# REXJJ/depth-map-fusion-utils

Hardware: AMD Instinct MI355X
Metric: ray-voxel updates/sec (3D-DDA log-odds fusion, 512^3 grid, 640x480 depth) (higher is better)
Workload: dtype int32

## Files before the change

### depth-map-fusion-utils_amd/csrc/dmf_dda.hpp

```cpp
#pragma once
#include "dmf_internal.hpp"

namespace dmf {

constexpr int64_t kQ = 256;

__device__ inline int64_t clampi(int64_t v, int64_t lo, int64_t hi) { return v < lo ? lo : (v > hi ? hi : v); }
__device__ inline int32_t clamp32(int32_t v, int32_t lo, int32_t hi) { return v < lo ? lo : (v > hi ? hi : v); }

__device__ inline int32_t floor_sat32(double x) {
  const double f = floor(x);
  return fabs(f) < 9223372036854775808.0 ? (int32_t)fmin(fmax(f, -1073741824.0), 1073741824.0) : -(1 << 30);
}

__device__ inline void atomic_add_dev(int32_t* p, int32_t v) {
  __hip_atomic_fetch_add(p, v, __ATOMIC_RELAXED, __HIP_MEMORY_SCOPE_AGENT);
}

struct Tiles {
  uint32_t ny, nz;
};
__host__ __device__ inline Tiles tiles_of(const int n[3]) {
  return Tiles{(uint32_t)(n[1] + 1) >> 1, (uint32_t)(n[2] + 3) >> 2};
}
__host__ __device__ inline uint32_t tile_base(const Tiles& t, int tx, int ty, int tz) {
  return (((uint32_t)tx * t.ny + (uint32_t)ty) * t.nz + (uint32_t)tz) << 4;
}
__host__ __device__ inline uint32_t tiled_index(const Tiles& t, int x, int y, int z) {
  return tile_base(t, x >> 1, y >> 1, z >> 2) | (uint32_t)(((x & 1) << 3) | ((y & 1) << 2) | (z & 3));
}
inline size_t tiled_cells(const int n[3]) {
  return (size_t)((n[0] + 1) >> 1) * (size_t)((n[1] + 1) >> 1) * (size_t)((n[2] + 3) >> 2) * 16;
}

struct Ray {
  int c[3];
  int st[3];
  int32_t E01, E02, E12;
  int32_t K[3];
  int left;
  bool end_inside;
};
constexpr int32_t kNever = 1 << 30;

__device__ inline void dda_select(int32_t& E01, int32_t& E02, int32_t& E12, int32_t K0, int32_t K1, int32_t K2,
                                  bool& s0, bool& s1, bool& s2) {
  const bool b10 = E01 > 0;
  s2 = (b10 ? E12 : E02) > 0;
  s1 = !s2 && b10;
  s0 = !s2 && !b10;
  E01 += s0 ? K1 : (s1 ? -K0 : 0);
  E02 += s0 ? K2 : (s2 ? -K0 : 0);
  E12 += s1 ? K2 : (s2 ? -K1 : 0);
}

__device__ inline double grid_coord(const Geom& g, int a, float x) {
  const double t = (double)x - g.mn[a];
  return g.pow2 ? t * g.inv[a] : t / g.dl[a];
}

__device__ inline void grid_origin(const Geom& g, const float O[3], double go[3]) {
#pragma unroll
  for (int a = 0; a < 3; ++a) go[a] = grid_coord(g, a, O[a]);
}

__device__ inline bool dda_quantize_go(const Geom& g, const double go[3], const float E[3], bool end_inside,
                                       int64_t qs[3], int64_t qe[3]) {
  double ge[3], D[3];
#pragma unroll
  for (int a = 0; a < 3; ++a) {
    ge[a] = grid_coord(g, a, E[a]);
    D[a] = ge[a] - go[a];
  }
  double t0 = 0.0, t1 = 1.0;
#pragma unroll
  for (int a = 0; a < 3; ++a) {
    if (D[a] == 0.0) {
      if (go[a] < 0.0 || go[a] >= (double)g.n[a]) return false;
    } else if (end_inside) {
      if (D[a] > 0.0 ? go[a] < 0.0 : go[a] > (double)g.n[a]) {
        const double lo = (D[a] > 0.0 ? 0.0 - go[a] : (double)g.n[a] - go[a]) / D[a];
        if (lo > t0) t0 = lo;
      }
    } else {
      double ta = (0.0 - go[a]) / D[a];
      double tb = ((double)g.n[a] - go[a]) / D[a];
      if (ta > tb) { const double tt = ta; ta = tb; tb = tt; }
      if (ta > t0) t0 = ta;
      if (tb < t1) t1 = tb;
    }
  }
  if (end_inside) { t1 = 1.0; if (t0 > 1.0) t0 = 1.0; }
  if (t0 > t1) return false;
#pragma unroll
  for (int a = 0; a < 3; ++a) {
    const double gs = go[a] + t0 * D[a];
    const double gx = end_inside ? ge[a] : go[a] + t1 * D[a];
    const int32_t n = (int32_t)g.n[a], Q = (int32_t)kQ;
    const int32_t cs = clamp32(floor_sat32(gs), 0, n - 1);
    const int32_t ce = end_inside ? floor_sat32(ge[a]) : clamp32(floor_sat32(gx), 0, n - 1);
    qs[a] = clamp32(floor_sat32(gs * (double)kQ), cs * Q, cs * Q + Q - 1);
    qe[a] = clamp32(floor_sat32(gx * (double)kQ), ce * Q, ce * Q + Q - 1);
  }
  return true;
}

__device__ inline bool dda_quantize(const Geom& g, const float O[3], const float E[3], bool end_inside, int64_t qs[3],
                                    int64_t qe[3]) {
  double go[3];
  grid_origin(g, O, go);
  return dda_quantize_go(g, go, E, end_inside, qs, qe);
}

__device__ inline bool dda_setup(const Geom& g, const float O[3], const float E[3], bool end_inside, Ray& R) {
  int64_t qs[3], qe[3];
  if (!dda_quantize(g, O, E, end_inside, qs, qe)) return false;
  int64_t cs[3], ce[3];
#pragma unroll
  for (int a = 0; a < 3; ++a) {
    cs[a] = qs[a] / kQ;
    ce[a] = qe[a] / kQ;
  }
  int64_t adq[3], h[3];
#pragma unroll
  for (int a = 0; a < 3; ++a) {
    const int64_t dq = qe[a] - qs[a];
    adq[a] = dq < 0 ? -dq : dq;
    R.st[a] = ce[a] > cs[a] ? 1 : (ce[a] < cs[a] ? -1 : 0);
    h[a] = R.st[a] > 0 ? 2 * ((cs[a] + 1) * kQ - qs[a]) : 2 * (qs[a] - cs[a] * kQ) + 1;
    R.K[a] = (int32_t)(2 * kQ * adq[a]);
  }
  auto pair = [&](int a, int b) -> int32_t {
    if (R.st[a] && R.st[b]) return (int32_t)(h[a] * adq[b] - h[b] * adq[a]);
    return R.st[a] ? -kNever : (R.st[b] ? kNever : 0);
  };
  R.E01 = pair(0, 1);
  R.E02 = pair(0, 2);
  R.E12 = pair(1, 2);
  const int nsteps = (int)((ce[0] > cs[0] ? ce[0] - cs[0] : cs[0] - ce[0]) + (ce[1] > cs[1] ? ce[1] - cs[1] : cs[1] - ce[1]) +
                           (ce[2] > cs[2] ? ce[2] - cs[2] : cs[2] - ce[2]));
  R.c[0] = (int)cs[0];
  R.c[1] = (int)cs[1];
  R.c[2] = (int)cs[2];
  R.left = nsteps + 1;
  R.end_inside = end_inside;
  return true;
}

__device__ inline bool endpoint_inside(const Geom& g, const float E[3]) {
  const bool in = (E[0] >= g.vlo[0]) & (E[0] <= g.vhi[0]) & (E[1] >= g.vlo[1]) & (E[1] <= g.vhi[1]) &
                  (E[2] >= g.vlo[2]) & (E[2] <= g.vhi[2]);
  if (!in) return false;
  return valid_coords(g, bin_axis(g, 0, E[0]), bin_axis(g, 1, E[1]), bin_axis(g, 2, E[2]));
}

__device__ inline int pixel_ray(const Geom& g, const CamP& cam, const uint16_t* __restrict__ depth,
                                const PoseX* __restrict__ poses, int p, int r, int c, int dmin, int dmax, Ray& R,
                                bool& valid) {
  R.left = 0;
  valid = false;
  if (r >= cam.H || c >= cam.W) return 0;
  const int d = depth[((int64_t)p * cam.H + r) * cam.W + c];
  if (!(d >= dmin && d < dmax)) return 0;
  valid = true;
  const PoseX& T = poses[p];
  float pc[3], E[3];
  project(cam, r, c, d, pc);
  xform(T.f, pc[0], pc[1], pc[2], E);
  const bool inside = endpoint_inside(g, E);
  const float O[3] = {T.f[3], T.f[7], T.f[11]};
  if (!dda_setup(g, O, E, inside, R)) { R.left = 0; return 0; }
  return R.left;
}

__device__ inline bool pixel_quant_go(const Geom& g, const CamP& cam, int d, const float Tf[12], const double go[3],
                                      int r, int c, int dmin, int dmax, int64_t qs[3], int64_t qe[3], bool& inside,
                                      bool& valid) {
  valid = false;
  inside = false;
  if (d < 0 || !(d >= dmin && d < dmax)) return false;
  valid = true;
  float pc[3], E[3];
  project(cam, r, c, d, pc);
  xform(Tf, pc[0], pc[1], pc[2], E);
  inside = endpoint_inside(g, E);
  return dda_quantize_go(g, go, E, inside, qs, qe);
}

__device__ inline int pixel_depth(const CamP& cam, const uint16_t* __restrict__ depth, int p, int r, int c) {
  return (r >= cam.H || c >= cam.W) ? -1 : (int)depth[((int64_t)p * cam.H + r) * cam.W + c];
}

}
```

### depth-map-fusion-utils_amd/csrc/dmf_fuse.hip

```cpp
#include <algorithm>
#include <atomic>
#include <cmath>
#include <cstdlib>
#include <string>
#include <type_traits>

#include "dmf_brick.hpp"
#include "dmf_dda.hpp"
#include "dmf_host.hpp"

namespace dmf {

struct DepthSrc {
  CamP cam;
  const uint16_t* depth;
  const PoseX* poses;
  int dmin, dmax, packets_x;
  struct Frame { float Tf[12]; };
  struct Sample { int d, r, c; };
  __device__ void begin(const Geom& g, int p, Frame& f, double go[3]) const {
#pragma unroll
    for (int i = 0; i < 12; ++i) f.Tf[i] = poses[p].f[i];
    const float O[3] = {f.Tf[3], f.Tf[7], f.Tf[11]};
    grid_origin(g, O, go);
// ... 21 lines not shown
  int64_t N;
  struct Frame { bool live; };
  struct Sample { float E[3]; bool ok; };
  __device__ static bool finite3(const float v[3]) {
    return __builtin_isfinite(v[0]) & __builtin_isfinite(v[1]) & __builtin_isfinite(v[2]);
  }
  __device__ void origin(int p, float O[3]) const {
    const float* const o = origins + 3 * (int64_t)p;
    O[0] = o[0];
    O[1] = o[1];
    O[2] = o[2];
  }
  __device__ void begin(const Geom& g, int p, Frame& f, double go[3]) const {
    float O[3];
    origin(p, O);
    f.live = finite3(O);
    grid_origin(g, O, go);
  }
  __device__ Sample load(int p, int q, int l) const {
    Sample s;
    const int64_t i = (int64_t)q * 64 + l;
    s.ok = i < N;
    const float* const e = xyz + ((int64_t)p * N + (s.ok ? i : 0)) * 3;
    s.E[0] = e[0];
    s.E[1] = e[1];
    s.E[2] = e[2];
    return s;
  }
  __device__ bool quant(const Geom& g, const Frame& f, const double go[3], const Sample& s, int64_t qs[3],
                        int64_t qe[3], bool& inside, bool& valid) const {
    inside = false;
    valid = f.live & s.ok & finite3(s.E);
    if (!valid) return false;
    inside = endpoint_inside(g, s.E);
    return dda_quantize_go(g, go, s.E, inside, qs, qe);
  }
  __device__ int ray(const Geom& g, int p, int q, int l, Ray& R, bool& valid) const {
    float O[3];
    origin(p, O);
    const Sample s = load(p, q, l);
    R.left = 0;
    valid = finite3(O) && s.ok && finite3(s.E);
    if (!valid) return 0;
    if (!dda_setup(g, O, s.E, endpoint_inside(g, s.E), R)) { R.left = 0; return 0; }
    return R.left;
  }
};

__device__ inline void wave_stats(unsigned long long* stats, unsigned long long upd, unsigned long long ray,
                                  unsigned long long hit) {
  for (int o = 32; o > 0; o >>= 1) {
    upd += __shfl_down(upd, o, 64);
    ray += __shfl_down(ray, o, 64);
    hit += __shfl_down(hit, o, 64);
  }
  if ((threadIdx.x & 63) == 0) {
    if (upd) atomicAdd(&stats[0], upd);
    if (ray) atomicAdd(&stats[1], ray);
    if (hit) atomicAdd(&stats[2], hit);
  }
}


typedef unsigned short us2 __attribute__((ext_vector_type(2)));
__device__ inline uint32_t pkmax(uint32_t a, uint32_t b) {
  us2 x = __builtin_bit_cast(us2, a), y = __builtin_bit_cast(us2, b);
  return __builtin_bit_cast(uint32_t, __builtin_elementwise_max(x, y));
}
__device__ inline uint32_t wave_pkmax(uint32_t v) {
  v = pkmax(v, (uint32_t)__builtin_amdgcn_update_dpp(0, (int)v, 0x111, 0xf, 0xf, false));
  v = pkmax(v, (uint32_t)__builtin_amdgcn_update_dpp(0, (int)v, 0x112, 0xf, 0xf, false));
  v = pkmax(v, (uint32_t)__builtin_amdgcn_update_dpp(0, (int)v, 0x114, 0xf, 0xf, false));
  v = pkmax(v, (uint32_t)__builtin_amdgcn_update_dpp(0, (int)v, 0x118, 0xf, 0xf, false));
  v = pkmax(v, (uint32_t)__builtin_amdgcn_update_dpp(0, (int)v, 0x142, 0xa, 0xf, false));
  v = pkmax(v, (uint32_t)__builtin_amdgcn_update_dpp(0, (int)v, 0x143, 0xc, 0xf, false));
  return (uint32_t)__builtin_amdgcn_readlane((int)v, 63);
}

__device__ inline int lane_prefix(uint64_t mask) {
  return (int)__builtin_amdgcn_mbcnt_hi((uint32_t)(mask >> 32), __builtin_amdgcn_mbcnt_lo((uint32_t)mask, 0u));
}

__device__ inline int small_div(int i, int b, float rb, int& rem) {
  int q = (int)((float)i * rb);
  int r = i - q * b;
  if (r < 0) { --q; r += b; }
  if (r >= b) { ++q; r -= b; }
  rem = r;
  return q;
}

__device__ inline int popc(uint32_t v) { return __builtin_popcount(v); }
__device__ inline int popc(uint64_t v) { return __builtin_popcountll(v); }

template <int kS, int kBox, class Src>
__global__ __launch_bounds__(64) void k_fuse_l(Geom g, Src src, int32_t* __restrict__ hits,
                                               int32_t* __restrict__ misses,
                                               unsigned long long* __restrict__ stats) {
  static_assert(kS <= 31, "2-bit codes of up to 31 advances with a 64-bit field mask");
  using CodeT = typename std::conditional<(kS <= 15), uint32_t, uint64_t>::type;
  constexpr CodeT kOne = 1, kOdd = (CodeT)0x5555555555555555ull, kEven = (CodeT)0xAAAAAAAAAAAAAAAAull;
  static_assert(kBox % 256 == 0 && kBox <= 65536, "box scanned 256 cells per iteration, 16-bit indices");
  static_assert(kBox >= 64 * kS, "the non-zero list lives in the box");
  stats = stat_slot(stats);
  __shared__ __attribute__((aligned(16))) int box[kBox];
  uint32_t* nzl = (uint32_t*)box;
  const int l = threadIdx.x;
  for (int i = l; i < kBox; i += 64) box[i] = 0;
  const Tiles tl = tiles_of(g.n);
  Ray R;
  bool valid;
  const unsigned long long upd = (unsigned long long)src.ray(g, (int)blockIdx.y, (int)blockIdx.x, l, R, valid);
  const unsigned long long nvalid = valid ? 1 : 0, nhit = (R.left > 0 && R.end_inside) ? 1 : 0;
  int32_t E01 = R.E01, E02 = R.E02, E12 = R.E12;
  const int32_t K0 = R.K[0], K1 = R.K[1], K2 = R.K[2];
  const int st0 = R.st[0], st1 = R.st[1], st2 = R.st[2];
  int c0 = R.c[0], c1 = R.c[1], c2 = R.c[2], left = R.left;
  const bool end_inside = R.end_inside;
  const int rot = ((l & 7) + 3 * (l >> 3)) % kS;
  unsigned long long nflush = 0, nround_lds = 0, nround_direct = 0;
  while (__builtin_amdgcn_ballot_w64(left > 0)) {
    const int rem = left < kS ? left : kS;
// ... 171 lines not shown

constexpr uint32_t kHashEmpty = 0xffff0000u;
__device__ inline bool hash_add(uint32_t* tab, uint32_t mask, int shift, uint32_t b, uint32_t n) {
  uint32_t h = (b * 2654435761u) >> shift;
  for (uint32_t k = 0; k <= mask; ++k) {
    const uint32_t old = atomicCAS(&tab[h], kHashEmpty, b << 16 | n);
    if (old == kHashEmpty) return true;
    if ((old >> 16) == b) {
      atomicAdd(&tab[h], n);
      return true;
    }
    h = (h + 1) & mask;
  }
  return false;
}

__device__ inline void hash_add_first(uint32_t* tab, uint32_t mask, int shift, int b, uint32_t* ovf) {
  const int b0 = __builtin_amdgcn_readfirstlane(b);
  const uint64_t same = __builtin_amdgcn_ballot_w64(b == b0);
  const int l = (int)(threadIdx.x & 63);
  if (b == b0 && l != __builtin_ctzll(same)) return;
  const uint32_t n = b == b0 ? (uint32_t)__builtin_popcountll(same) : 1u;
  if (!hash_add(tab, mask, shift, (uint32_t)b, n)) *ovf = 1u;
}

template <class Src>
struct BkRaysArgs {
  Geom g;
  Src src;
  int packets_pose, wg_pose, span;
  BkGeom bg;
  ulonglong2* rays;
  uint64_t* paths;
  uint32_t* pose_cnt;
  uint32_t* wg_base;
  uint32_t* wg_list;
  int wgl_stride;
  unsigned long long* pose_pairs;
  unsigned long long* stats;
  uint32_t* ovl;
  int hash_log;
};

template <bool H16, bool HASH, class Src>
__device__ inline void bk_rays_wg(const BkRaysArgs<Src>& A_, unsigned wg, uint32_t* hist, uint32_t* sh) {
  const Geom& g = A_.g;
  const BkGeom& bg = A_.bg;
  unsigned long long* const stats = stat_slot(A_.stats);
  const uint32_t hmask = (1u << A_.hash_log) - 1u;
  const int hshift = 32 - A_.hash_log;
  if (threadIdx.x == 0) {
    sh[0] = 0;
    sh[1] = 0;
  }
  const int nwords = HASH ? (int)hmask + 1 : (H16 ? (bg.nbricks + 1) >> 1 : bg.nbricks);
  for (int i = threadIdx.x; i < nwords; i += blockDim.x) hist[i] = HASH ? kHashEmpty : 0u;
  __syncthreads();
  const int w = threadIdx.x >> 6, l = threadIdx.x & 63, nw = blockDim.x >> 6;
  const int pw = (int)(wg / (unsigned)A_.wg_pose);
  const int q0 = (int)(wg - (unsigned)pw * (unsigned)A_.wg_pose) * A_.span;
  const int64_t pk0 = (int64_t)pw * A_.packets_pose + q0,
                pk1 = (int64_t)pw * A_.packets_pose + min(A_.packets_pose, q0 + A_.span);
  unsigned long long upd = 0, nvalid = 0, nhit = 0;
  double go[3];
  typename Src::Frame fr;
  A_.src.begin(g, pw, fr, go);
  for (int64_t pk = pk0 + w; pk < pk1; pk += nw) {
    const int p = pw;
    const int q = (int)(pk - (int64_t)p * A_.packets_pose);
    const typename Src::Sample sm = A_.src.load(p, q, l);
    int64_t qs[3], qe[3];
    bool inside, valid;
    ulonglong2 rec;
    rec.x = 0;
    rec.y = 0;
    uint64_t path = 0;
    if (A_.src.quant(g, fr, go, sm, qs, qe, inside, valid)) {
      uint64_t A, B;
      bk::pack_ray(qs, qe, inside, A, B);
      rec.x = A;
      rec.y = B;
      bk::QRay R;
      const int32_t qs32[3] = {(int32_t)qs[0], (int32_t)qs[1], (int32_t)qs[2]},
                    qe32[3] = {(int32_t)qe[0], (int32_t)qe[1], (int32_t)qe[2]};
      bk::qray_from(qs32, qe32, inside, R);
      upd += (unsigned long long)(R.nsteps + 1);
      nhit += inside ? 1 : 0;
      path = bk_coarse(bg, R, [&](int b) {
        if constexpr (HASH) hash_add_first(hist, hmask, hshift, b, &sh[1]);
        else hist_add_first<H16>(hist, b);
      });
    }
    nvalid += valid ? 1 : 0;
    A_.rays[pk * 64 + l] = rec;
    A_.paths[pk * 64 + l] = path;
  }
  __syncthreads();
  if (HASH && sh[1]) {
    if (threadIdx.x == 0) A_.ovl[1 + atomicAdd(&A_.ovl[0], 1u)] = wg;
    return;
  }
  uint32_t* const pc = A_.pose_cnt + (size_t)pw * bg.nbricks;
  uint32_t* const row = A_.wg_list + (size_t)wg * (size_t)A_.wgl_stride;
  unsigned long long mine = 0;
  for (int i = threadIdx.x; i < nwords; i += blockDim.x) {
    uint32_t b, n;
    if constexpr (HASH) {
      const uint32_t e = hist[i];
      b = e >> 16;
      n = e == kHashEmpty ? 0u : (e & 0xffffu);
    } else {
      b = (uint32_t)i;
      n = hist[i];
    }
    if (!HASH && H16) {
      for (int hh = 0; hh < 2; ++hh) {
        const uint32_t bb = 2u * (uint32_t)i + (uint32_t)hh, nn = (n >> (16 * hh)) & 0xffffu;
        if (nn) {
          A_.wg_base[(size_t)wg * bg.nbricks + bb] = atomicAdd(&pc[bb], nn);
          const uint32_t k = atomicAdd(&sh[0], 1u);
          row[1 + k] = bb | nn << 16;
          mine += nn;
        }
      }
    } else if (n) {
      A_.wg_base[(size_t)wg * bg.nbricks + b] = atomicAdd(&pc[b], n);
      const uint32_t k = atomicAdd(&sh[0], 1u);
      row[1 + k] = b | n << 16;
// ... 284 lines not shown
      s_bt[0] = J;
      for (uint32_t k = 0; k <= J + 1; ++k) bt[k] = s_bt[k];
    }
  }
  if (j > 0) {
    const uint32_t J = bt[0];
    for (uint32_t k = t; k <= J + 1 && k < kBkLayout1Poses + 2; k += blockDim.x) s_bt[k] = bt[k];
  }
  __syncthreads();
  if ((uint32_t)j >= s_bt[0]) {
    if (t == 0) ctl[0] = ctl[1] = ctl[2] = ctl[3] = 0;
    return;
  }
  const int p0 = (int)s_bt[1 + j], p1 = (int)s_bt[2 + j];
  for (int b = t; b < nbricks; b += blockDim.x) {
    const uint32_t acc = bk_pose_prefix(pose_cnt, pose_base, nbricks, b, p0, p1);
    cnt[b] = acc;
    s_cnt[b] = acc;
  }
  __syncthreads();
  bk_scan_body<false>(nbricks, cnt, s_cnt, off, part_pref, ctl, order, part_max, split_cu);
}

constexpr uint32_t kBkSlotSentinel = 0xF0000000u;
__device__ inline uint32_t bk_e30(int32_t e) {
  const int32_t lim = (1 << 29) - 1;
  return (uint32_t)(e > lim ? lim : (e < -lim ? -lim : e)) & 0x3fffffffu;
}

template <bool SLAB>
__global__ __launch_bounds__(kBkPassThreadsBig) void k_bk_pairs(int packets_pose, int wg_pose, int span, BkGeom bg,
                                                         const ulonglong2* __restrict__ rays,
                                                         const uint64_t* __restrict__ paths,
                                                         const uint32_t* __restrict__ off,
                                                         const uint32_t* __restrict__ pose_base,
                                                         const uint32_t* __restrict__ wg_base,
                                                         const uint32_t* __restrict__ bt, int j,
                                                         const uint32_t* __restrict__ wg_list, int wgl_stride,
                                                         uint4* __restrict__ pa, void* __restrict__ pbv,
                                                         unsigned long long* __restrict__ ctl,
                                                         uint32_t* __restrict__ fault, int inject,
                                                         unsigned long long* __restrict__ stats) {
  uint2* const pb = (uint2*)pbv;
  uint32_t* const pw = (uint32_t*)pbv;
  extern __shared__ uint32_t hist[];
  const int pz = (int)(blockIdx.x / (unsigned)wg_pose);
  if ((uint32_t)j >= bt[0] || (uint32_t)pz < bt[1 + j] || (uint32_t)pz >= bt[2 + j]) return;
  const uint32_t total = (uint32_t)ctl[0];
  uint32_t extra = (inject > 0 && j == 0 && (uint32_t)pz == bt[1] && threadIdx.x == 0) ? (uint32_t)inject : 0u;
  const uint32_t* wb = wg_base + (size_t)blockIdx.x * bg.nbricks;
  const uint32_t* pbz = pose_base + (size_t)pz * bg.nbricks;
  {
    const uint32_t* row = wg_list + (size_t)blockIdx.x * (size_t)wgl_stride;
    const uint32_t nl = row[0];
    for (int i = threadIdx.x; i < bg.nbricks; i += blockDim.x) hist[i] = kBkSlotSentinel;
    __syncthreads();
    for (uint32_t k = threadIdx.x; k < nl; k += blockDim.x) {
      const int i = (int)(row[1 + k] & 0xffffu);
      hist[i] = off[i] + pbz[i] + wb[i];
    }
  }
  __syncthreads();
  uint32_t over = 0;
#if defined(DMF_EXP_STATS)
  unsigned long long b_iters = 0, b_lanes = 0;
#endif
  const int w = threadIdx.x >> 6, l = threadIdx.x & 63, nw = blockDim.x >> 6;
  const int q0 = (int)(blockIdx.x - (unsigned)pz * (unsigned)wg_pose) * span;
  const int64_t pk0 = (int64_t)pz * packets_pose + q0, pk1 = (int64_t)pz * packets_pose + min(packets_pose, q0 + span);
  constexpr uint32_t m5 = bk::kB - 1;
  ulonglong2 rnext = make_ulonglong2(0, 0);
  uint64_t pnext = 0;
  if (pk0 + w < pk1) {
    rnext = rays[(pk0 + w) * 64 + l];
    pnext = paths[(pk0 + w) * 64 + l];
  }
  for (int64_t pk = pk0 + w; pk < pk1; pk += nw) {
    const ulonglong2 rec = rnext;
    const uint64_t path = pnext;
    if (pk + nw < pk1) {
      rnext = rays[(pk + nw) * 64 + l];
      pnext = paths[(pk + nw) * 64 + l];
    }
    if ((rec.y >> 63) == 0) continue;
    bk::QRay R;
    bk::decode_ray(rec.x, rec.y, R);
    const uint32_t K0 = (uint32_t)(2 * bk::kQ) * (uint32_t)R.adq[0], K1 = (uint32_t)(2 * bk::kQ) * (uint32_t)R.adq[1],
                   K2 = (uint32_t)(2 * bk::kQ) * (uint32_t)R.adq[2];
    const uint32_t e01 = (uint32_t)bk::e0_pair(R, 0, 1), e02 = (uint32_t)bk::e0_pair(R, 0, 2),
                   e12 = (uint32_t)bk::e0_pair(R, 1, 2);
    const uint32_t signs = (R.st[0] < 0 ? 1u << 22 : 0u) | (R.st[1] < 0 ? 1u << 23 : 0u) | (R.st[2] < 0 ? 1u << 24 : 0u);
    const int M = SLAB ? bk::major_axis(R) : 0;
    const int m1 = M == 0 ? 1 : 0, m2 = M == 2 ? 1 : 2;
    const uint32_t aM = (uint32_t)bk::pick3(R.adq[0], R.adq[1], R.adq[2], M),
                   a1 = (uint32_t)bk::pick3(R.adq[0], R.adq[1], R.adq[2], m1),
                   a2 = (uint32_t)bk::pick3(R.adq[0], R.adq[1], R.adq[2], m2);
    const uint32_t KM = (uint32_t)(2 * bk::kQ) * aM, Km1 = (uint32_t)(2 * bk::kQ) * a1, Km2 = (uint32_t)(2 * bk::kQ) * a2;
    int32_t sb1 = 0, sb2 = 0, sb12 = 0;
    if (SLAB) bk::slab_from_pairwise(M, (int32_t)e01, (int32_t)e02, (int32_t)e12, sb1, sb2, sb12);
    const uint2 wb0 = make_uint2((uint32_t)R.adq[0] | (((uint32_t)R.adq[2] & 0x3fffu) << 18),
                                 (uint32_t)R.adq[1] | (((uint32_t)R.adq[2] >> 14) << 18) | signs);
    auto entry = [&](const int32_t c[3]) {
      uint4 e;
      if (SLAB) {
        const uint32_t cM = (uint32_t)bk::pick3(c[0], c[1], c[2], M), c1 = (uint32_t)bk::pick3(c[0], c[1], c[2], m1),
                       c2 = (uint32_t)bk::pick3(c[0], c[1], c[2], m2);
        constexpr uint32_t k2 = (uint32_t)(2 * bk::kQ);
        auto m = [](uint32_t c, uint32_t a) { return (uint32_t)bk::mul24((int32_t)c, (int32_t)a); };
        e.x = (uint32_t)sb1 + (m(cM, a1) - m(c1, aM)) * k2;
        e.y = (uint32_t)sb2 + (m(cM, a2) - m(c2, aM)) * k2;
        e.z = (uint32_t)sb12 + (m(c1, a2) - m(c2, a1)) * k2;
      } else {
        e.x = e01 + (uint32_t)c[0] * K1 - (uint32_t)c[1] * K0;
        e.y = e02 + (uint32_t)c[0] * K2 - (uint32_t)c[2] * K0;
        e.z = e12 + (uint32_t)c[1] * K2 - (uint32_t)c[2] * K1;
      }
      const uint32_t x = (uint32_t)(R.cs[0] + bk::mul24(R.st[0], c[0])) & m5,
// ... 594 lines not shown
  int64_t max_batches(int64_t P) const { return (P / PS) * jmax(PS) + (P % PS ? jmax(P % PS) : 0); }
  int split_cu = 0;
  size_t max_parts() const { return (size_t)bg.nbricks + pair_cap / part_max + 1 + 3 * 1024; }
};

static int64_t cam_packets(const CamP& cp) { return (int64_t)((cp.W + 7) / 8) * ((cp.H + 7) / 8); }
static int64_t scan_packets(int64_t N) { return (N + 63) / 64; }

static int bk_plan(const dmf_volume* v, int64_t ppose, const Geom& g, int P, BkPlan& pl) {
  const int64_t* kn = v->knob;
  pl.bg = brick_geom(g);
  pl.ppose = ppose;
  pl.max_pairs_ray = 1 + (pl.bg.nb[0] - 1) + (pl.bg.nb[1] - 1) + (pl.bg.nb[2] - 1);
  pl.rec_bytes = v->fuse_variant == DMF_FUSE_CELL_WALK ? 24 : 20;
  const int64_t rays_pose = pl.ppose * 64;
  const uint64_t one_pose = (uint64_t)rays_pose * (uint64_t)pl.max_pairs_ray;
  if (one_pose > (uint64_t)UINT32_MAX) return fail(DMF_ERR_RANGE, "one frame exceeds the 32-bit pair offsets");
  pl.ab_threads = pl.bg.nbricks > kBkBigHist ? kBkPassThreadsBig : kBkPassThreads;
  pl.span = std::max((pl.bg.nbricks <= 512 ? 8 : 16) * (pl.ab_threads / 64), (pl.bg.nbricks + 63) / 64);
  if (kn[DMF_KNOB_A_HASH] > 0) {
    int lg = 4;
    while (lg < 14 && (1ll << lg) < kn[DMF_KNOB_A_HASH]) ++lg;
    pl.hash_log = lg;
  } else if (kn[DMF_KNOB_A_HASH] == 0 && pl.bg.nbricks > kBkBigHist) {
    pl.hash_log = 11;
    pl.span = 128;
  }
  if (kn[DMF_KNOB_SPAN] > 0) pl.span = (int)std::max<int64_t>(4, std::min<int64_t>(kn[DMF_KNOB_SPAN], 1023));
  if (kn[DMF_KNOB_PART_MAX] > 0)
    pl.part_max = (uint32_t)std::max<int64_t>(1024, std::min<int64_t>(kn[DMF_KNOB_PART_MAX], kBkPartMax));
  pl.wg_pose = (int)((pl.ppose + pl.span - 1) / pl.span);
  pl.hist_bytes = sizeof(uint32_t) * (size_t)pl.bg.nbricks;
  pl.wgl_stride = 1 + pl.bg.nbricks;
  pl.per_pose_bytes = (uint64_t)rays_pose * (sizeof(ulonglong2) + sizeof(uint64_t)) + (uint64_t)pl.wg_pose * pl.hist_bytes +
                      (uint64_t)pl.wg_pose * sizeof(uint32_t) * (uint64_t)pl.wgl_stride + 2 * (uint64_t)pl.hist_bytes +
                      sizeof(unsigned long long) + sizeof(uint32_t);
  pl.slots = v->pipelined ? 2 : 1;
  const uint64_t budget = v->bk_budget / (uint64_t)pl.slots;
  pl.PS = std::min<int64_t>(P, (int64_t)(budget / 2 / pl.per_pose_bytes));
  if (kn[DMF_KNOB_SUPER_POSES] > 0) pl.PS = std::min<int64_t>(pl.PS, kn[DMF_KNOB_SUPER_POSES]);
  if (pl.PS < 1) return fail(DMF_ERR_RANGE, "one frame exceeds the brick fusion budget (dmf_fuse_reserve)");
  pl.pair_cap = std::min<uint64_t>({(budget - (uint64_t)pl.PS * pl.per_pose_bytes) / pl.rec_bytes,
                                    (uint64_t)pl.PS * one_pose, (uint64_t)kBkSlotSentinel - 1});
  if (pl.pair_cap < one_pose) return fail(DMF_ERR_RANGE, "one frame exceeds the brick fusion pair budget (dmf_fuse_reserve)");
  if (kn[DMF_KNOB_PAIR_CAP] > 0)
    pl.pair_cap = std::min<uint64_t>(pl.pair_cap, (uint64_t)kn[DMF_KNOB_PAIR_CAP]);
  pl.max_poses = (int)pl.PS;
  if (kn[DMF_KNOB_BATCH_POSES] > 0) pl.max_poses = (int)std::min<int64_t>(pl.PS, kn[DMF_KNOB_BATCH_POSES]);
  pl.PBg = std::max<int64_t>(1, std::min<int64_t>(pl.max_poses, (int64_t)(pl.pair_cap / one_pose)));
  const int64_t ts = kn[DMF_KNOB_TAIL_SPLIT];
  if (v->fuse_variant != DMF_FUSE_CELL_WALK && ts >= 0 && (ts > 0 || !v->pipelined)) {
    const int k = ts > 0 ? (int)std::min<int64_t>(ts, 8) : 2;
    pl.split_cu = std::min(512, cu_count(v->device)) | (k << 16);
  }
  pl.slot_bytes = pl.pair_cap * pl.rec_bytes + (uint64_t)pl.PS * pl.per_pose_bytes +
                  sizeof(uint32_t) * (3 * (uint64_t)pl.bg.nbricks + 6 + 2 * pl.max_parts()) +
                  sizeof(unsigned long long) * 4;
  return DMF_OK;
}

static int bk_attributes() {
  static std::atomic<bool> attr_set{false};
  if (!attr_set.load()) {
    const int lds = (int)(sizeof(uint32_t) * 32768);
    DMF_HIP(hipFuncSetAttribute((const void*)k_bk_rays<true, DepthSrc>, hipFuncAttributeMaxDynamicSharedMemorySize, lds));
    DMF_HIP(hipFuncSetAttribute((const void*)k_bk_rays_recover<DepthSrc>, hipFuncAttributeMaxDynamicSharedMemorySize, lds));
    DMF_HIP(hipFuncSetAttribute((const void*)k_bk_rays_hash<DepthSrc>, hipFuncAttributeMaxDynamicSharedMemorySize, lds));
    DMF_HIP(hipFuncSetAttribute((const void*)k_bk_rays<true, PointSrc>, hipFuncAttributeMaxDynamicSharedMemorySize, lds));
    DMF_HIP(hipFuncSetAttribute((const void*)k_bk_rays_recover<PointSrc>, hipFuncAttributeMaxDynamicSharedMemorySize, lds));
    DMF_HIP(hipFuncSetAttribute((const void*)k_bk_rays_hash<PointSrc>, hipFuncAttributeMaxDynamicSharedMemorySize, lds));
    DMF_HIP(hipFuncSetAttribute((const void*)k_bk_pairs<false>, hipFuncAttributeMaxDynamicSharedMemorySize, lds));
    DMF_HIP(hipFuncSetAttribute((const void*)k_bk_pairs<true>, hipFuncAttributeMaxDynamicSharedMemorySize, lds));
    attr_set.store(true);
  }
  return DMF_OK;
}

struct BkBufs {
  ulonglong2* rays = nullptr;
  uint64_t* paths = nullptr;
  uint32_t *cnt = nullptr, *off = nullptr, *part_pref = nullptr, *wgb = nullptr, *wgl = nullptr;
  uint32_t *pose_cnt = nullptr, *pose_base = nullptr, *bt = nullptr;
  unsigned long long* pose_pairs = nullptr;
  uint2* order = nullptr;
  unsigned long long* ctl = nullptr;
  uint4* pra = nullptr;
  void* prb = nullptr;
  uint32_t* ovl = nullptr;
};

static int bk_scratch(dmf_volume* v, const BkPlan& pl, BkBufs& b, int slot) {
  const size_t PS = (size_t)pl.PS, nb = (size_t)pl.bg.nbricks;
  void *rays, *bricks, *ctl, *wgb, *wgl, *pra, *prb, *pcnt, *pbase, *batch;
  const size_t nrays = (size_t)(pl.PS * pl.ppose * 64);
  DMF_TRY(scratch(v, slot ? kScBkRays1 : kScBkRays, (sizeof(ulonglong2) + sizeof(uint64_t)) * nrays, &rays));
  DMF_TRY(scratch(v, slot ? kScBkBricks1 : kScBkBricks, sizeof(uint32_t) * (3 * nb + 6 + 2 * pl.max_parts()), &bricks));
  DMF_TRY(scratch(v, slot ? kScBkCtl1 : kScBkCtl, sizeof(unsigned long long) * 4, &ctl));
  DMF_TRY(scratch(v, slot ? kScBkWgBase1 : kScBkWgBase, pl.hist_bytes * (size_t)pl.wg_pose * PS, &wgb));
  DMF_TRY(scratch(v, slot ? kScBkWgList1 : kScBkWgList,
                  sizeof(uint32_t) * (size_t)pl.wgl_stride * (size_t)pl.wg_pose * PS, &wgl));
  DMF_TRY(scratch(v, slot ? kScBkPairs1 : kScBkPairs, sizeof(uint4) * ((size_t)pl.pair_cap + 1), &pra));
  DMF_TRY(scratch(v, slot ? kScBkPairsB1 : kScBkPairsB, (pl.rec_bytes - sizeof(uint4)) * ((size_t)pl.pair_cap + 1),
                  &prb));
  DMF_TRY(scratch(v, slot ? kScBkPoseCnt1 : kScBkPoseCnt, pl.hist_bytes * PS, &pcnt));
  DMF_TRY(scratch(v, slot ? kScBkPoseBase1 : kScBkPoseBase, pl.hist_bytes * PS, &pbase));
  DMF_TRY(scratch(v, slot ? kScBkBatch1 : kScBkBatch, sizeof(unsigned long long) * PS + sizeof(uint32_t) * (PS + 4),
                  &batch));
  void* ovl;
  DMF_TRY(scratch(v, slot ? kScBkOvf1 : kScBkOvf, sizeof(uint32_t) * (1 + (size_t)pl.wg_pose * PS), &ovl));
  b.ovl = (uint32_t*)ovl;
  b.rays = (ulonglong2*)rays;
  b.paths = (uint64_t*)(b.rays + nrays);
  b.cnt = (uint32_t*)bricks;
  b.off = b.cnt + nb;
  b.part_pref = b.off + nb;
  b.order = (uint2*)(b.part_pref + nb + 4 + (nb & 1));
  b.wgb = (uint32_t*)wgb;
  b.wgl = (uint32_t*)wgl;
  b.ctl = (unsigned long long*)ctl;
  b.pra = (uint4*)pra;
  b.prb = prb;
  b.pose_cnt = (uint32_t*)pcnt;
  b.pose_base = (uint32_t*)pbase;
  b.pose_pairs = (unsigned long long*)batch;
  b.bt = (uint32_t*)(b.pose_pairs + PS);
  return DMF_OK;
}

static int bk_release(dmf_volume* v) {
  static const int kSlots[] = {kScBkRays, kScBkPairs, kScBkPairsB, kScBkBricks, kScBkWgBase, kScBkCtl, kScBkPoseCnt,
                               kScBkPoseBase, kScBkBatch, kScBkWgList, kScBkRays1, kScBkWgBase1, kScBkWgList1,
                               kScBkPoseCnt1, kScBkBatch1, kScBkBricks1, kScBkCtl1, kScBkPairs1, kScBkPairsB1,
                               kScBkPoseBase1, kScBkOvf, kScBkOvf1};
  if (v->stream) DMF_HIP(hipStreamSynchronize(v->stream));
  if (v->stage) DMF_HIP(hipStreamSynchronize(v->stage));
  for (int k : kSlots) {
    if (k < (int)v->scratch.size() && v->scratch[k].first) {
      DMF_HIP(hipFree(v->scratch[k].first));
      v->scratch[k] = {nullptr, 0};
    }
  }
  v->bk_last_bt = nullptr;
  return DMF_OK;
}

// ... 42 lines not shown
    }
    out = Src{cp, d_depth + (size_t)s0 * cp.H * cp.W, tab_a, dmin, dmax, (cp.W + 7) / 8};
    return DMF_OK;
  }
};
struct PointFeed {
  using Src = PointSrc;
  const float* d_xyz;
  const float* d_origins;
  int64_t N;
  int64_t packets() const { return scan_packets(N); }
  int source(dmf_volume*, int64_t s0, int64_t, int64_t, bool, int, hipStream_t, Src& out) const {
    out = Src{d_xyz + (size_t)s0 * (size_t)N * 3, d_origins + (size_t)s0 * 3, N};
    return DMF_OK;
  }
};

template <class Feed>
static int fuse_bricks(dmf_volume* v, const Feed& feed, const Geom& g, int P, int32_t* d_hits, int32_t* d_misses,
                       unsigned long long* st, uint64_t* d_user, bool staged, bool capturing) {
  using Src = typename Feed::Src;
  BkPlan pl;
  DMF_TRY(bk_plan(v, feed.packets(), g, P, pl));
  const BkGeom& bg = pl.bg;
  DMF_TRY(bk_attributes());
  DMF_TRY(fault_words(v));
  BkBufs b;
  if (staged) DMF_TRY(stage_init(v));
  const bool slab = v->fuse_variant != DMF_FUSE_CELL_WALK;
  if ((int64_t)pl.span * 64 > 65535) return fail(DMF_ERR_RANGE, "pass A span %d exceeds 16-bit counts", pl.span);
  const unsigned nf = (unsigned)cu_count(v->device);
  auto pass_b = [&](auto kernel, unsigned nwg, hipStream_t s, int64_t j) {
    hipLaunchKernelGGL(kernel, dim3(nwg), dim3(pl.ab_threads), pl.hist_bytes, s, (int)pl.ppose, pl.wg_pose, pl.span, bg,
                       (const ulonglong2*)b.rays, (const uint64_t*)b.paths, (const uint32_t*)b.off,
                       (const uint32_t*)b.pose_base, (const uint32_t*)b.wgb, (const uint32_t*)b.bt, (int)j,
                       (const uint32_t*)b.wgl, pl.wgl_stride, b.pra, b.prb, b.ctl, v->d_fault,
                       (int)std::min<int64_t>(v->knob[DMF_KNOB_FAULT_INJECT], 1 << 20), st);
  };
  auto scan = [&](auto kernel, hipStream_t s, int64_t j) {
    hipLaunchKernelGGL(kernel, dim3(1), dim3(1024), 0, s, bg.nbricks, (const uint32_t*)b.cnt, b.off, b.part_pref, b.ctl,
                       b.order, pl.part_max, (const uint32_t*)b.bt, (int)j, pl.split_cu);
  };
  for (int64_t s0 = 0; s0 < P; s0 += pl.PS) {
    const int64_t ps = std::min<int64_t>(pl.PS, P - s0);
    const unsigned nwg = (unsigned)(ps * pl.wg_pose);
    const int slot = staged ? v->st_slot : 0;
    DMF_TRY(bk_scratch(v, pl, b, slot));
    const hipStream_t sa = staged ? v->stage : v->stream;
    unsigned long long* st_a = st;
    if (staged) {
      v->st_slot ^= 1;
      DMF_HIP(hipEventRecord(v->st_in, v->in_stream));
      DMF_HIP(hipStreamWaitEvent(sa, v->st_in, 0));
      if (v->st_free_set[slot]) DMF_HIP(hipStreamWaitEvent(sa, v->st_free[slot], 0));
    }
    Src src;
    DMF_TRY(feed.source(v, s0, ps, pl.PS, staged, slot, sa, src));
    if (staged) {
      if (st) {
        void* sbuf;
        DMF_TRY(scratch(v, slot ? kScStStats1 : kScStStats0, sizeof(unsigned long long) * kStatSlots * kStatWidth, &sbuf));
        DMF_HIP(hipMemsetAsync(sbuf, 0, sizeof(unsigned long long) * kStatSlots * kStatWidth, sa));
        st_a = (unsigned long long*)sbuf;
      }
    }
    DMF_HIP(hipMemsetAsync(b.pose_cnt, 0, pl.hist_bytes * (size_t)ps, sa));
    DMF_HIP(hipMemsetAsync(b.pose_pairs, 0, sizeof(unsigned long long) * (size_t)ps, sa));
    if (staged && v->st_b_set[slot ^ 1]) DMF_HIP(hipStreamWaitEvent(sa, v->st_b_ev[slot ^ 1], 0));
    BkRaysArgs<Src> ra{g, src, (int)pl.ppose, pl.wg_pose, pl.span, bg, b.rays, b.paths, b.pose_cnt, b.wgb, b.wgl,
                       pl.wgl_stride, b.pose_pairs, st_a, b.ovl, 0};
    if (pl.hash_log > 0) {
      ra.hash_log = pl.hash_log;
      DMF_HIP(hipMemsetAsync(b.ovl, 0, sizeof(uint32_t), sa));
      hipLaunchKernelGGL(k_bk_rays_hash<Src>, dim3(nwg), dim3(kBkPassThreads), sizeof(uint32_t) << pl.hash_log, sa, ra);
      DMF_LAUNCH_CHECK();
      hipLaunchKernelGGL(k_bk_rays_recover<Src>, dim3(nf), dim3(kBkPassThreadsBig),
                         sizeof(uint32_t) * ((bg.nbricks + 1) / 2), sa, ra);
    } else {
      hipLaunchKernelGGL((k_bk_rays<true, Src>), dim3(nwg), dim3(pl.ab_threads),
                         sizeof(uint32_t) * ((bg.nbricks + 1) / 2), sa, ra);
    }
    DMF_LAUNCH_CHECK();
    if (staged) {
      DMF_HIP(hipEventRecord(v->st_a[slot], sa));
      DMF_HIP(hipStreamWaitEvent(v->stream, v->st_a[slot], 0));
      if (st) DMF_TRY(stats_end(v, st_a, d_user, kStatWidth, nullptr, sa));
      DMF_HIP(hipEventRecord(v->st_done[slot], sa));
      DMF_HIP(hipStreamWaitEvent(v->in_stream, v->st_done[slot], 0));
    }
    const hipStream_t sl = v->stream;
    const bool layout1 = bg.nbricks <= kBkLayout1Bricks && ps <= kBkLayout1Poses;
    if (!layout1) {
      hipLaunchKernelGGL(k_bk_batches, dim3(1), dim3(1024), 0, sl, (int)ps, (const unsigned long long*)b.pose_pairs,
                         (unsigned long long)pl.pair_cap, pl.max_poses, b.bt);
      DMF_LAUNCH_CHECK();
    }
    v->bk_last_bt = b.bt;
    const int64_t jm = pl.jmax(ps);
    for (int64_t j = 0; j < jm; ++j) {
      const hipStream_t sj = sl;
      if (layout1) {
        hipLaunchKernelGGL(k_bk_layout1, dim3(1), dim3(1024), 0, sj, (int)ps, (const unsigned long long*)b.pose_pairs,
                           (unsigned long long)pl.pair_cap, pl.max_poses, b.bt, bg.nbricks, (int)j,
// ... 520 lines not shown
```

Before: 1530 billion.

## Skip empty ray packets via wave ballot masks and share endpoint grid coords

Result: no change. 1541 billion, median of 6 (+0.7%).

```diff
diff --git a/depth-map-fusion-utils_amd/csrc/dmf_dda.hpp b/depth-map-fusion-utils_amd/csrc/dmf_dda.hpp
--- a/depth-map-fusion-utils_amd/csrc/dmf_dda.hpp
+++ b/depth-map-fusion-utils_amd/csrc/dmf_dda.hpp
@@ -1,17 +1,10 @@
 #pragma once
 #include "dmf_internal.hpp"
+#include "dmf_quant.hpp"
 
 namespace dmf {
 
-constexpr int64_t kQ = 256;
-
 __device__ inline int64_t clampi(int64_t v, int64_t lo, int64_t hi) { return v < lo ? lo : (v > hi ? hi : v); }
-__device__ inline int32_t clamp32(int32_t v, int32_t lo, int32_t hi) { return v < lo ? lo : (v > hi ? hi : v); }
-
-__device__ inline int32_t floor_sat32(double x) {
-  const double f = floor(x);
-  return fabs(f) < 9223372036854775808.0 ? (int32_t)fmin(fmax(f, -1073741824.0), 1073741824.0) : -(1 << 30);
-}
 
 __device__ inline void atomic_add_dev(int32_t* p, int32_t v) {
   __hip_atomic_fetch_add(p, v, __ATOMIC_RELAXED, __HIP_MEMORY_SCOPE_AGENT);
@@ -54,55 +47,12 @@
   E12 += s1 ? K2 : (s2 ? -K1 : 0);
 }
 
-__device__ inline double grid_coord(const Geom& g, int a, float x) {
-  const double t = (double)x - g.mn[a];
-  return g.pow2 ? t * g.inv[a] : t / g.dl[a];
-}
-
-__device__ inline void grid_origin(const Geom& g, const float O[3], double go[3]) {
-#pragma unroll
-  for (int a = 0; a < 3; ++a) go[a] = grid_coord(g, a, O[a]);
-}
-
 __device__ inline bool dda_quantize_go(const Geom& g, const double go[3], const float E[3], bool end_inside,
                                        int64_t qs[3], int64_t qe[3]) {
-  double ge[3], D[3];
+  double ge[3];
 #pragma unroll
-  for (int a = 0; a < 3; ++a) {
-    ge[a] = grid_coord(g, a, E[a]);
-    D[a] = ge[a] - go[a];
-  }
-  double t0 = 0.0, t1 = 1.0;
-#pragma unroll
-  for (int a = 0; a < 3; ++a) {
-    if (D[a] == 0.0) {
-      if (go[a] < 0.0 || go[a] >= (double)g.n[a]) return false;
-    } else if (end_inside) {
-      if (D[a] > 0.0 ? go[a] < 0.0 : go[a] > (double)g.n[a]) {
-        const double lo = (D[a] > 0.0 ? 0.0 - go[a] : (double)g.n[a] - go[a]) / D[a];
-        if (lo > t0) t0 = lo;
-      }
-    } else {
-      double ta = (0.0 - go[a]) / D[a];
-      double tb = ((double)g.n[a] - go[a]) / D[a];
-      if (ta > tb) { const double tt = ta; ta = tb; tb = tt; }
-      if (ta > t0) t0 = ta;
-      if (tb < t1) t1 = tb;
-    }
-  }
-  if (end_inside) { t1 = 1.0; if (t0 > 1.0) t0 = 1.0; }
-  if (t0 > t1) return false;
-#pragma unroll
-  for (int a = 0; a < 3; ++a) {
-    const double gs = go[a] + t0 * D[a];
-    const double gx = end_inside ? ge[a] : go[a] + t1 * D[a];
-    const int32_t n = (int32_t)g.n[a], Q = (int32_t)kQ;
-    const int32_t cs = clamp32(floor_sat32(gs), 0, n - 1);
-    const int32_t ce = end_inside ? floor_sat32(ge[a]) : clamp32(floor_sat32(gx), 0, n - 1);
-    qs[a] = clamp32(floor_sat32(gs * (double)kQ), cs * Q, cs * Q + Q - 1);
-    qe[a] = clamp32(floor_sat32(gx * (double)kQ), ce * Q, ce * Q + Q - 1);
-  }
-  return true;
+  for (int a = 0; a < 3; ++a) ge[a] = grid_coord(g, a, E[a]);
+  return dda_quantize_at(g, go, ge, end_inside, qs, qe);
 }
 
 __device__ inline bool dda_quantize(const Geom& g, const float O[3], const float E[3], bool end_inside, int64_t qs[3],
@@ -148,10 +98,10 @@
 }
 
 __device__ inline bool endpoint_inside(const Geom& g, const float E[3]) {
-  const bool in = (E[0] >= g.vlo[0]) & (E[0] <= g.vhi[0]) & (E[1] >= g.vlo[1]) & (E[1] <= g.vhi[1]) &
-                  (E[2] >= g.vlo[2]) & (E[2] <= g.vhi[2]);
-  if (!in) return false;
-  return valid_coords(g, bin_axis(g, 0, E[0]), bin_axis(g, 1, E[1]), bin_axis(g, 2, E[2]));
+  double ge[3];
+#pragma unroll
+  for (int a = 0; a < 3; ++a) ge[a] = grid_coord(g, a, E[a]);
+  return endpoint_inside_at(g, E, ge);
 }
 
 __device__ inline int pixel_ray(const Geom& g, const CamP& cam, const uint16_t* __restrict__ depth,
@@ -183,8 +133,7 @@
   float pc[3], E[3];
   project(cam, r, c, d, pc);
   xform(Tf, pc[0], pc[1], pc[2], E);
-  inside = endpoint_inside(g, E);
-  return dda_quantize_go(g, go, E, inside, qs, qe);
+  return dda_quantize_end(g, go, E, qs, qe, inside);
 }
 
 __device__ inline int pixel_depth(const CamP& cam, const uint16_t* __restrict__ depth, int p, int r, int c) {
diff --git a/depth-map-fusion-utils_amd/csrc/dmf_fuse.hip b/depth-map-fusion-utils_amd/csrc/dmf_fuse.hip
--- a/depth-map-fusion-utils_amd/csrc/dmf_fuse.hip
+++ b/depth-map-fusion-utils_amd/csrc/dmf_fuse.hip
@@ -77,8 +77,7 @@
     inside = false;
     valid = f.live & s.ok & finite3(s.E);
     if (!valid) return false;
-    inside = endpoint_inside(g, s.E);
-    return dda_quantize_go(g, go, s.E, inside, qs, qe);
+    return dda_quantize_end(g, go, s.E, qs, qe, inside);
   }
   __device__ int ray(const Geom& g, int p, int q, int l, Ray& R, bool& valid) const {
     float O[3];
@@ -133,6 +132,12 @@
   if (r >= b) { ++q; r -= b; }
   rem = r;
   return q;
+}
+
+__device__ inline uint64_t wave_u64(uint64_t v) {
+  const uint32_t lo = (uint32_t)__builtin_amdgcn_readfirstlane((int)(uint32_t)v),
+                 hi = (uint32_t)__builtin_amdgcn_readfirstlane((int)(uint32_t)(v >> 32));
+  return (uint64_t)hi << 32 | lo;
 }
 
 __device__ inline int popc(uint32_t v) { return __builtin_popcount(v); }
@@ -370,6 +375,7 @@
   BkGeom bg;
   ulonglong2* rays;
   uint64_t* paths;
+  uint64_t* masks;
   uint32_t* pose_cnt;
   uint32_t* wg_base;
   uint32_t* wg_list;
@@ -430,8 +436,12 @@
       });
     }
     nvalid += valid ? 1 : 0;
-    A_.rays[pk * 64 + l] = rec;
-    A_.paths[pk * 64 + l] = path;
+    const uint64_t mask = __builtin_amdgcn_ballot_w64((rec.y >> 63) != 0);
+    if (l == 0) A_.masks[pk] = mask;
+    if (mask) {
+      A_.rays[pk * 64 + l] = rec;
+      A_.paths[pk * 64 + l] = path;
+    }
   }
   __syncthreads();
   if (HASH && sh[1]) {
@@ -782,6 +792,7 @@
 __global__ __launch_bounds__(kBkPassThreadsBig) void k_bk_pairs(int packets_pose, int wg_pose, int span, BkGeom bg,
                                                          const ulonglong2* __restrict__ rays,
                                                          const uint64_t* __restrict__ paths,
+                                                         const uint64_t* __restrict__ masks,
                                                          const uint32_t* __restrict__ off,
                                                          const uint32_t* __restrict__ pose_base,
                                                          const uint32_t* __restrict__ wg_base,
@@ -821,18 +832,24 @@
   constexpr uint32_t m5 = bk::kB - 1;
   ulonglong2 rnext = make_ulonglong2(0, 0);
   uint64_t pnext = 0;
-  if (pk0 + w < pk1) {
+  uint64_t mnext = 0, mnext2 = 0;
+  if (pk0 + w < pk1) mnext = wave_u64(masks[pk0 + w]);
+  if (pk0 + w + nw < pk1) mnext2 = masks[pk0 + w + nw];
+  if (mnext) {
     rnext = rays[(pk0 + w) * 64 + l];
     pnext = paths[(pk0 + w) * 64 + l];
   }
   for (int64_t pk = pk0 + w; pk < pk1; pk += nw) {
     const ulonglong2 rec = rnext;
     const uint64_t path = pnext;
-    if (pk + nw < pk1) {
+    const uint64_t mask = mnext;
+    mnext = wave_u64(mnext2);
+    mnext2 = pk + 2 * nw < pk1 ? masks[pk + 2 * nw] : 0;
+    if (mnext) {
       rnext = rays[(pk + nw) * 64 + l];
       pnext = paths[(pk + nw) * 64 + l];
     }
-    if ((rec.y >> 63) == 0) continue;
+    if (!((mask >> l) & 1)) continue;
     bk::QRay R;
     bk::decode_ray(rec.x, rec.y, R);
     const uint32_t K0 = (uint32_t)(2 * bk::kQ) * (uint32_t)R.adq[0], K1 = (uint32_t)(2 * bk::kQ) * (uint32_t)R.adq[1],
@@ -1493,7 +1510,8 @@
   pl.wg_pose = (int)((pl.ppose + pl.span - 1) / pl.span);
   pl.hist_bytes = sizeof(uint32_t) * (size_t)pl.bg.nbricks;
   pl.wgl_stride = 1 + pl.bg.nbricks;
-  pl.per_pose_bytes = (uint64_t)rays_pose * (sizeof(ulonglong2) + sizeof(uint64_t)) + (uint64_t)pl.wg_pose * pl.hist_bytes +
+  pl.per_pose_bytes = (uint64_t)rays_pose * (sizeof(ulonglong2) + sizeof(uint64_t)) +
+                      (uint64_t)pl.ppose * sizeof(uint64_t) + (uint64_t)pl.wg_pose * pl.hist_bytes +
                       (uint64_t)pl.wg_pose * sizeof(uint32_t) * (uint64_t)pl.wgl_stride + 2 * (uint64_t)pl.hist_bytes +
                       sizeof(unsigned long long) + sizeof(uint32_t);
   pl.slots = v->pipelined ? 2 : 1;
@@ -1540,6 +1558,7 @@
 struct BkBufs {
   ulonglong2* rays = nullptr;
   uint64_t* paths = nullptr;
+  uint64_t* masks = nullptr;
   uint32_t *cnt = nullptr, *off = nullptr, *part_pref = nullptr, *wgb = nullptr, *wgl = nullptr;
   uint32_t *pose_cnt = nullptr, *pose_base = nullptr, *bt = nullptr;
   unsigned long long* pose_pairs = nullptr;
@@ -1553,8 +1572,9 @@
 static int bk_scratch(dmf_volume* v, const BkPlan& pl, BkBufs& b, int slot) {
   const size_t PS = (size_t)pl.PS, nb = (size_t)pl.bg.nbricks;
   void *rays, *bricks, *ctl, *wgb, *wgl, *pra, *prb, *pcnt, *pbase, *batch;
-  const size_t nrays = (size_t)(pl.PS * pl.ppose * 64);
-  DMF_TRY(scratch(v, slot ? kScBkRays1 : kScBkRays, (sizeof(ulonglong2) + sizeof(uint64_t)) * nrays, &rays));
+  const size_t nrays = (size_t)(pl.PS * pl.ppose * 64), npackets = (size_t)(pl.PS * pl.ppose);
+  DMF_TRY(scratch(v, slot ? kScBkRays1 : kScBkRays,
+                  (sizeof(ulonglong2) + sizeof(uint64_t)) * nrays + sizeof(uint64_t) * npackets, &rays));
   DMF_TRY(scratch(v, slot ? kScBkBricks1 : kScBkBricks, sizeof(uint32_t) * (3 * nb + 6 + 2 * pl.max_parts()), &bricks));
   DMF_TRY(scratch(v, slot ? kScBkCtl1 : kScBkCtl, sizeof(unsigned long long) * 4, &ctl));
   DMF_TRY(scratch(v, slot ? kScBkWgBase1 : kScBkWgBase, pl.hist_bytes * (size_t)pl.wg_pose * PS, &wgb));
@@ -1572,6 +1592,7 @@
   b.ovl = (uint32_t*)ovl;
   b.rays = (ulonglong2*)rays;
   b.paths = (uint64_t*)(b.rays + nrays);
+  b.masks = b.paths + nrays;
   b.cnt = (uint32_t*)bricks;
   b.off = b.cnt + nb;
   b.part_pref = b.off + nb;
@@ -1680,8 +1701,9 @@
   const unsigned nf = (unsigned)cu_count(v->device);
   auto pass_b = [&](auto kernel, unsigned nwg, hipStream_t s, int64_t j) {
     hipLaunchKernelGGL(kernel, dim3(nwg), dim3(pl.ab_threads), pl.hist_bytes, s, (int)pl.ppose, pl.wg_pose, pl.span, bg,
-                       (const ulonglong2*)b.rays, (const uint64_t*)b.paths, (const uint32_t*)b.off,
-                       (const uint32_t*)b.pose_base, (const uint32_t*)b.wgb, (const uint32_t*)b.bt, (int)j,
+                       (const ulonglong2*)b.rays, (const uint64_t*)b.paths, (const uint64_t*)b.masks,
+                       (const uint32_t*)b.off, (const uint32_t*)b.pose_base, (const uint32_t*)b.wgb,
+                       (const uint32_t*)b.bt, (int)j,
                        (const uint32_t*)b.wgl, pl.wgl_stride, b.pra, b.prb, b.ctl, v->d_fault,
                        (int)std::min<int64_t>(v->knob[DMF_KNOB_FAULT_INJECT], 1 << 20), st);
   };
@@ -1715,8 +1737,8 @@
     DMF_HIP(hipMemsetAsync(b.pose_cnt, 0, pl.hist_bytes * (size_t)ps, sa));
     DMF_HIP(hipMemsetAsync(b.pose_pairs, 0, sizeof(unsigned long long) * (size_t)ps, sa));
     if (staged && v->st_b_set[slot ^ 1]) DMF_HIP(hipStreamWaitEvent(sa, v->st_b_ev[slot ^ 1], 0));
-    BkRaysArgs<Src> ra{g, src, (int)pl.ppose, pl.wg_pose, pl.span, bg, b.rays, b.paths, b.pose_cnt, b.wgb, b.wgl,
-                       pl.wgl_stride, b.pose_pairs, st_a, b.ovl, 0};
+    BkRaysArgs<Src> ra{g, src, (int)pl.ppose, pl.wg_pose, pl.span, bg, b.rays, b.paths, b.masks, b.pose_cnt, b.wgb,
+                       b.wgl, pl.wgl_stride, b.pose_pairs, st_a, b.ovl, 0};
     if (pl.hash_log > 0) {
       ra.hash_log = pl.hash_log;
       DMF_HIP(hipMemsetAsync(b.ovl, 0, sizeof(uint32_t), sa));
diff --git a/depth-map-fusion-utils_amd/csrc/dmf_quant.hpp b/depth-map-fusion-utils_amd/csrc/dmf_quant.hpp
--- /dev/null
+++ b/depth-map-fusion-utils_amd/csrc/dmf_quant.hpp
@@ -0,0 +1,86 @@
+#pragma once
+#include "dmf_geom.hpp"
+
+namespace dmf {
+
+constexpr int64_t kQ = 256;
+
+__host__ __device__ inline int32_t clamp32(int32_t v, int32_t lo, int32_t hi) { return v < lo ? lo : (v > hi ? hi : v); }
+
+__host__ __device__ inline int32_t floor_sat32(double x) {
+  const double f = floor(x);
+  return fabs(f) < 9223372036854775808.0 ? (int32_t)fmin(fmax(f, -1073741824.0), 1073741824.0) : -(1 << 30);
+}
+
+__host__ __device__ inline int32_t cell_sat32(int32_t f, double x) {
+  const uint32_t hi = (uint32_t)(__builtin_bit_cast(uint64_t, x) >> 32);
+  return hi - 0x43600000u < 0x00800000u ? 1 << 30 : f >> 8;
+}
+
+__host__ __device__ inline double grid_coord(const Geom& g, int a, float x) {
+  const double t = (double)x - g.mn[a];
+  return g.pow2 ? t * g.inv[a] : t / g.dl[a];
+}
+
+__host__ __device__ inline void grid_origin(const Geom& g, const float O[3], double go[3]) {
+#pragma unroll
+  for (int a = 0; a < 3; ++a) go[a] = grid_coord(g, a, O[a]);
+}
+
+__host__ __device__ inline bool endpoint_inside_at(const Geom& g, const float E[3], const double ge[3]) {
+  const bool in = (E[0] >= g.vlo[0]) & (E[0] <= g.vhi[0]) & (E[1] >= g.vlo[1]) & (E[1] <= g.vhi[1]) &
+                  (E[2] >= g.vlo[2]) & (E[2] <= g.vhi[2]);
+  if (!in) return false;
+  const int x = (int)floor(ge[0]), y = (int)floor(ge[1]), z = (int)floor(ge[2]);
+  return x < g.n[0] && y < g.n[1] && z < g.n[2] && x >= 0 && y >= 0 && z >= 0;
+}
+
+__host__ __device__ inline bool dda_quantize_at(const Geom& g, const double go[3], const double ge[3],
+                                                bool end_inside, int64_t qs[3], int64_t qe[3]) {
+  double D[3];
+#pragma unroll
+  for (int a = 0; a < 3; ++a) D[a] = ge[a] - go[a];
+  double t0 = 0.0, t1 = 1.0;
+#pragma unroll
+  for (int a = 0; a < 3; ++a) {
+    if (D[a] == 0.0) {
+      if (go[a] < 0.0 || go[a] >= (double)g.n[a]) return false;
+    } else if (end_inside) {
+      if (D[a] > 0.0 ? go[a] < 0.0 : go[a] > (double)g.n[a]) {
+        const double lo = (D[a] > 0.0 ? 0.0 - go[a] : (double)g.n[a] - go[a]) / D[a];
+        if (lo > t0) t0 = lo;
+      }
+    } else {
+      double ta = (0.0 - go[a]) / D[a];
+      double tb = ((double)g.n[a] - go[a]) / D[a];
+      if (ta > tb) { const double tt = ta; ta = tb; tb = tt; }
+      if (ta > t0) t0 = ta;
+      if (tb < t1) t1 = tb;
+    }
+  }
+  if (end_inside) { t1 = 1.0; if (t0 > 1.0) t0 = 1.0; }
+  if (t0 > t1) return false;
+#pragma unroll
+  for (int a = 0; a < 3; ++a) {
+    const double gs = go[a] + t0 * D[a];
+    const double gx = end_inside ? ge[a] : go[a] + t1 * D[a];
+    const int32_t n = (int32_t)g.n[a], Q = (int32_t)kQ;
+    const int32_t fs = floor_sat32(gs * (double)kQ), fx = floor_sat32(gx * (double)kQ);
+    const int32_t cs = clamp32(cell_sat32(fs, gs), 0, n - 1);
+    const int32_t ce = end_inside ? fx >> 8 : clamp32(cell_sat32(fx, gx), 0, n - 1);
+    qs[a] = clamp32(fs, cs * Q, cs * Q + Q - 1);
+    qe[a] = clamp32(fx, ce * Q, ce * Q + Q - 1);
+  }
+  return true;
+}
+
+__host__ __device__ inline bool dda_quantize_end(const Geom& g, const double go[3], const float E[3], int64_t qs[3],
+                                                 int64_t qe[3], bool& inside) {
+  double ge[3];
+#pragma unroll
+  for (int a = 0; a < 3; ++a) ge[a] = grid_coord(g, a, E[a]);
+  inside = endpoint_inside_at(g, E, ge);
+  return dda_quantize_at(g, go, ge, inside, qs, qe);
+}
+
+}
```
